# QZ1-boy/FCVSR

Hardware: AMD Instinct MI355X
Metric: SR frames/sec (7-frame window, 4x 180x320->720x1280) + PSNR vs ref (higher is better)
Workload: dtype bf16

## Files before the change

fcvsr_amd/csrc/iac.hip:

```cpp
#include "common.h"
#include "mfma_util.h"

namespace fcvsr {

typedef __attribute__((ext_vector_type(4))) float f32x4v_t;

constexpr int kIY = 4, kIX = 16, kIC = 32;
constexpr int kIHX = kIX + 2, kIHY = kIY + 2;

template <int KDT>
__device__ __forceinline__ void load_k12(const void* base, long long elem_off, float k[4][3]) {
  if (KDT == FCVSR_F32) {
    const float4* p = reinterpret_cast<const float4*>(reinterpret_cast<const float*>(base) + elem_off);
    const float4 a = p[0], b = p[1], c = p[2];
    k[0][0] = a.x; k[0][1] = a.y; k[0][2] = a.z; k[1][0] = a.w; k[1][1] = b.x; k[1][2] = b.y;
    k[2][0] = b.z; k[2][1] = b.w; k[2][2] = c.x; k[3][0] = c.y; k[3][1] = c.z; k[3][2] = c.w;
  } else {
    const uint2* p = reinterpret_cast<const uint2*>(reinterpret_cast<const uint16_t*>(base) + elem_off);
    const uint2 a = p[0], b = p[1], c = p[2];
    const unsigned w[6] = {a.x, a.y, b.x, b.y, c.x, c.y};
    float f[12];
#pragma unroll
    for (int i = 0; i < 6; ++i) {
      if (KDT == FCVSR_BF16) {
        f[2 * i] = __uint_as_float(w[i] << 16);
        f[2 * i + 1] = __uint_as_float(w[i] & 0xffff0000u);
      } else {
        typedef __attribute__((ext_vector_type(2))) _Float16 h2;
        const h2 hv = __builtin_bit_cast(h2, w[i]);
        f[2 * i] = (float)hv[0];
        f[2 * i + 1] = (float)hv[1];
      }
    }
#pragma unroll
    for (int c = 0; c < 4; ++c)
#pragma unroll
      for (int t = 0; t < 3; ++t) k[c][t] = f[c * 3 + t];
  }
}

template <int ADT>
__device__ __forceinline__ float4 ld_f4(const float* base, long long elem) {
  if (ADT == FCVSR_F32) return *reinterpret_cast<const float4*>(base + elem);
  const uint2 v = *reinterpret_cast<const uint2*>(reinterpret_cast<const uint16_t*>(base) + elem);
  if (ADT == FCVSR_BF16)
    return make_float4(__uint_as_float(v.x << 16), __uint_as_float(v.x & 0xffff0000u), __uint_as_float(v.y << 16),
                       __uint_as_float(v.y & 0xffff0000u));
  typedef __attribute__((ext_vector_type(2))) _Float16 h2;
  const h2 a = __builtin_bit_cast(h2, v.x), b = __builtin_bit_cast(h2, v.y);
  return make_float4((float)a[0], (float)a[1], (float)b[0], (float)b[1]);
}

template <int ADT>
__device__ __forceinline__ void st_f4(float* base, long long elem, float4 x) {
  if (ADT == FCVSR_F32) {
    *reinterpret_cast<float4*>(base + elem) = x;
  } else if (ADT == FCVSR_BF16) {
    typedef __attribute__((ext_vector_type(4))) __bf16 b4;
    const b4 c = {(__bf16)x.x, (__bf16)x.y, (__bf16)x.z, (__bf16)x.w};
    *reinterpret_cast<uint2*>(reinterpret_cast<uint16_t*>(base) + elem) = __builtin_bit_cast(uint2, c);
  } else {
    typedef __attribute__((ext_vector_type(4))) _Float16 h4;
    const h4 c = {(_Float16)x.x, (_Float16)x.y, (_Float16)x.z, (_Float16)x.w};
    *reinterpret_cast<uint2*>(reinterpret_cast<uint16_t*>(base) + elem) = __builtin_bit_cast(uint2, c);
  }
}

template <int KDT, int ADT>
__global__ __launch_bounds__(256) void iac_step_kernel(View prev, View off, View k1, View fin, float slope, int B, int H,
                                                       int W, View dst, int tiles_x, int tiles_y) {
  __shared__ __align__(16) float s_s[kIHY * kIHX * kIC];
  __shared__ __align__(16) float v_s[kIY * kIHX * kIC];
  const int tid = threadIdx.x;
  const int quad = tid & 7;
  const int c0 = blockIdx.y * kIC + quad * 4;
  const int t = blockIdx.x;
  const int b = t / (tiles_x * tiles_y);
  const int t2 = t - b * tiles_x * tiles_y;
  const int ty0 = (t2 / tiles_x) * kIY, tx0 = (t2 % tiles_x) * kIX;

  const long long pp = (long long)b * prev.sb + c0;
  for (int hp = tid >> 3; hp < kIHY * kIHX; hp += 32) {
    const int hy = hp / kIHX, hx = hp - hy * kIHX;
    int gy = ty0 + hy - 1, gx = tx0 + hx - 1;
    gy = gy < 0 ? 0 : (gy > H - 1 ? H - 1 : gy);
    gx = gx < 0 ? 0 : (gx > W - 1 ? W - 1 : gx);
    const float* op = off.p + (long long)b * off.sb + (long long)gy * off.sy + (long long)gx * off.sx;
    const float fx = (float)gx + op[0];
    const float fy = (float)gy + op[off.sc];
    const float x0f = floorf(fx), y0f = floorf(fy);
    const float wx1 = fx - x0f, wy1 = fy - y0f;
    const float wx0 = 1.f - wx1, wy0 = 1.f - wy1;
    const bool sane = (fx > -2.f) && (fx < (float)W + 1.f) && (fy > -2.f) && (fy < (float)H + 1.f);
    const int x0 = sane ? (int)x0f : -4, y0 = sane ? (int)y0f : -4;
    float4 acc = make_float4(0.f, 0.f, 0.f, 0.f);
#pragma unroll
    for (int dy = 0; dy < 2; ++dy) {
#pragma unroll
      for (int dx = 0; dx < 2; ++dx) {
        const int xi = x0 + dx, yi = y0 + dy;
        if (xi >= 0 && xi < W && yi >= 0 && yi < H) {
          const float w = (dy ? wy1 : wy0) * (dx ? wx1 : wx0);
          const float4 v = ld_f4<ADT>(prev.p, pp + (long long)yi * prev.sy + (long long)xi * prev.sx);
          acc.x = fmaf(v.x, w, acc.x); acc.y = fmaf(v.y, w, acc.y);
          acc.z = fmaf(v.z, w, acc.z); acc.w = fmaf(v.w, w, acc.w);
        }
      }
    }
    *reinterpret_cast<float4*>(s_s + hp * kIC + quad * 4) = acc;
  }
  __syncthreads();

  for (int vp = tid >> 3; vp < kIY * kIHX; vp += 32) {
    const int y = vp / kIHX, hx = vp - y * kIHX;
    int gy = ty0 + y, gx = tx0 + hx - 1;
    gy = gy > H - 1 ? H - 1 : gy;
    gx = gx < 0 ? 0 : (gx > W - 1 ? W - 1 : gx);
    float k[4][3];
    load_k12<KDT>(k1.p, (long long)b * k1.sb + (long long)gy * k1.sy + (long long)gx * k1.sx + c0 * 3, k);
    float4 acc = make_float4(0.f, 0.f, 0.f, 0.f);
#pragma unroll
    for (int tt = 0; tt < 3; ++tt) {
      const float4 v = *reinterpret_cast<const float4*>(s_s + ((y + tt) * kIHX + hx) * kIC + quad * 4);
      acc.x = fmaf(v.x, k[0][tt], acc.x); acc.y = fmaf(v.y, k[1][tt], acc.y);
      acc.z = fmaf(v.z, k[2][tt], acc.z); acc.w = fmaf(v.w, k[3][tt], acc.w);
    }
    *reinterpret_cast<float4*>(v_s + vp * kIC + quad * 4) = acc;
  }
  __syncthreads();

  for (int p = tid >> 3; p < kIY * kIX; p += 32) {
    const int y = p / kIX, x = p - y * kIX;
    const int gy = ty0 + y, gx = tx0 + x;
    if (gy < H && gx < W) {
      float k[4][3];
      load_k12<KDT>(k1.p, (long long)b * k1.sb + (long long)gy * k1.sy + (long long)gx * k1.sx + c0 * 3, k);
      float4 acc = make_float4(0.f, 0.f, 0.f, 0.f);
#pragma unroll
      for (int tt = 0; tt < 3; ++tt) {
        const float4 v = *reinterpret_cast<const float4*>(v_s + (y * kIHX + x + tt) * kIC + quad * 4);
        acc.x = fmaf(v.x, k[0][tt], acc.x); acc.y = fmaf(v.y, k[1][tt], acc.y);
        acc.z = fmaf(v.z, k[2][tt], acc.z); acc.w = fmaf(v.w, k[3][tt], acc.w);
      }
      const float4 f = ld_f4<ADT>(fin.p, (long long)b * fin.sb + (long long)gy * fin.sy + (long long)gx * fin.sx + c0);
      acc.x += f.x; acc.y += f.y; acc.z += f.z; acc.w += f.w;
      acc.x = acc.x >= 0.f ? acc.x : acc.x * slope; acc.y = acc.y >= 0.f ? acc.y : acc.y * slope;
      acc.z = acc.z >= 0.f ? acc.z : acc.z * slope; acc.w = acc.w >= 0.f ? acc.w : acc.w * slope;
      st_f4<ADT>(dst.p, (long long)b * dst.sb + (long long)gy * dst.sy + (long long)gx * dst.sx + c0, acc);
    }
  }
}

// ... 293 lines not shown
    for (int it = 0; it < NP; ++it) {
      const int src = dir * 32 + it * 8 + (lane >> 3);
#pragma unroll
      for (int q = 0; q < 4; ++q) {
        tap[dir][it][q] = ld_p8<ADT>(pb, __shfl(my_eo[q], src));
      }
    }
  };
  auto warp_store = [&](const int dir) {
#pragma unroll
    for (int it = 0; it < NP; ++it) {
      const int hp = it * 32 + ps;
      const int src = dir * 32 + it * 8 + (lane >> 3);
      float acc[8] = {0.f, 0.f, 0.f, 0.f, 0.f, 0.f, 0.f, 0.f};
      float tw[4];
#pragma unroll
      for (int q = 0; q < 4; ++q) tw[q] = __shfl(my_w[q], src);
#pragma unroll
      for (int q = 0; q < 4; ++q) {
        float v[8];
        unpack8<ADT>(tap[dir][it][q], v);
        const float w = tw[q];
#pragma unroll
        for (int c = 0; c < 8; ++c) acc[c] = fmaf(v[c], w, acc[c]);
      }
      if (hp < kIHY * kIHX) {
        *reinterpret_cast<float4*>(s_s + rec(hp, 0)) = make_float4(acc[0], acc[1], acc[2], acc[3]);
        *reinterpret_cast<float4*>(s_s + rec(hp, 1)) = make_float4(acc[4], acc[5], acc[6], acc[7]);
      }
    }
  };
  auto sac_phases = [&](const int dir) {
    const View dst = a.d[dir].dst;
#pragma unroll
    for (int j = 0; j < 3; ++j) {
      int y, hx;
      if (j < 2) { const int p = j * 32 + ps; y = p >> 4; hx = (p & 15) + 1; }
      else { y = ps >> 1; hx = (ps & 1) ? kIHX - 1 : 0; }
      if (j < 2 || ps < 8) {
        float k[24];
        unpack_k24<KDT>(j < 2 ? kin[j] : khal, k);
        float acc[8] = {0.f, 0.f, 0.f, 0.f, 0.f, 0.f, 0.f, 0.f};
#pragma unroll
        for (int tt = 0; tt < 3; ++tt) {
          const int sp = (y + tt) * kIHX + hx;
          const float4 va = *reinterpret_cast<const float4*>(s_s + rec(sp, 0)), vb = *reinterpret_cast<const float4*>(s_s + rec(sp, 1));
          const float v[8] = {va.x, va.y, va.z, va.w, vb.x, vb.y, vb.z, vb.w};
#pragma unroll
          for (int c = 0; c < 8; ++c) acc[c] = fmaf(v[c], k[c * 3 + tt], acc[c]);
        }
        const int vp = y * kIHX + hx;
        *reinterpret_cast<float4*>(v_s + rec(vp, 0)) = make_float4(acc[0], acc[1], acc[2], acc[3]);
        *reinterpret_cast<float4*>(v_s + rec(vp, 1)) = make_float4(acc[4], acc[5], acc[6], acc[7]);
      }
    }
    __syncthreads();
#pragma unroll
    for (int j = 0; j < 2; ++j) {
      const int p = j * 32 + ps;
      const int y = p >> 4, x = p & 15;
      const int gy = ty0 + y, gx = tx0 + x;
      if (gy < H && gx < W) {
        float k[24], f[8];
        unpack_k24<KDT>(kin[j], k);
        unpack8<ADT>(fpk[dir][j], f);
        float acc[8] = {0.f, 0.f, 0.f, 0.f, 0.f, 0.f, 0.f, 0.f};
#pragma unroll
        for (int tt = 0; tt < 3; ++tt) {
          const int vp = y * kIHX + x + tt;
          const float4 va = *reinterpret_cast<const float4*>(v_s + rec(vp, 0)), vb = *reinterpret_cast<const float4*>(v_s + rec(vp, 1));
          const float v[8] = {va.x, va.y, va.z, va.w, vb.x, vb.y, vb.z, vb.w};
#pragma unroll
          for (int c = 0; c < 8; ++c) acc[c] = fmaf(v[c], k[c * 3 + tt], acc[c]);
        }
#pragma unroll
        for (int c = 0; c < 8; ++c) {
          acc[c] += f[c];
          acc[c] = acc[c] >= 0.f ? acc[c] : acc[c] * slope;
        }
        st_p8<ADT>(dst.p, (long long)b * dst.sb + (long long)gy * dst.sy + (long long)gx * dst.sx + c0, acc);
      }
    }
  };

  issue_taps(0);
  if (FK) {
    predictor_gemm();
    __syncthreads();
#pragma unroll
    for (int j = 0; j < 2; ++j) {
      const int p = j * 32 + ps;
      const uint4* kq = reinterpret_cast<const uint4*>(kt_s + ((p >> 4) * kIHX + (p & 15) + 1) * kKtRow + oct * 24);
      kin[j].q[0] = kq[0]; kin[j].q[1] = kq[1]; kin[j].q[2] = kq[2];
    }
    if (ps < 8) {
      const uint4* kq = reinterpret_cast<const uint4*>(kt_s + ((ps >> 1) * kIHX + ((ps & 1) ? kIHX - 1 : 0)) * kKtRow + oct * 24);
      khal.q[0] = kq[0]; khal.q[1] = kq[1]; khal.q[2] = kq[2];
    }
    __syncthreads();
  }
  warp_store(0);
  if (ND > 1) { issue_taps(1); issue_fin(1); }
  if (t + 1 < t_end) off_next = load_off(t + 1, tid);
  __syncthreads();
  sac_phases(0);
  if (ND > 1) {
    warp_store(1);
    __syncthreads();
    sac_phases(1);
  }
  }
}


constexpr int kQX = 14, kQVX = 16, kQY = 4, kQSY = kQY + 2;
constexpr int kQNS = kQSY * kQVX, kQNV = kQY * kQVX;

template <bool BF16>
__device__ __forceinline__ f32x4v_t mfma16x(uint4 a, uint4 b, f32x4v_t c) {
  if (BF16)
    return __builtin_amdgcn_mfma_f32_16x16x32_bf16(__builtin_bit_cast(bf16x8_t, a), __builtin_bit_cast(bf16x8_t, b), c, 0, 0, 0);
  else
    return __builtin_amdgcn_mfma_f32_16x16x32_f16(__builtin_bit_cast(f16x8_t, a), __builtin_bit_cast(f16x8_t, b), c, 0, 0, 0);
}

struct Iac2Args {
  const uint16_t* prev[2];
  const float* off[2];
  const uint16_t* fin[2];
  uint16_t* dst[2];
  const uint16_t* k0;
  const uint16_t* wk;
  const float* kbias;
  long long prev_sb, off_sb, fin_sb, dst_sb, k0_sb;
  int prev_sy, prev_sx, off_sy, off_sx, off_sc, fin_sy, fin_sx, dst_sy, dst_sx, k0_sy, k0_sx;
  float slope;
  int H, W, tiles_x, tiles_y, ntiles;
};

#ifndef FCVSR_IAC2_WGS
#define FCVSR_IAC2_WGS 3
#endif
template <int KDT, int ADT>
__global__ __launch_bounds__(256, FCVSR_IAC2_WGS) void iac_fused2_kernel(Iac2Args a) {
  constexpr int NG = 1;
  static_assert(ADT != FCVSR_F32 && KDT != FCVSR_F32, "16-bit form");
  constexpr bool BF = KDT == FCVSR_BF16;
  constexpr int SPP = 32 * NG;
  constexpr int ND = 2, NP = (kQNS + SPP - 1) / SPP;
  constexpr int EARLY = 2;
  __shared__ __align__(16) float s_all[kQNS * kJC];
  __shared__ __align__(16) uint16_t w_s[3 * kJC * kJC];
  __shared__ __align__(16) float kb_s[3 * kJC];
  const float slope = a.slope;
  const int H = a.H, W = a.W, tiles_x = a.tiles_x, tiles_y = a.tiles_y;
  int t_begin, t_end;
  {
    const int g = blockIdx.x, nwg = gridDim.x, qq = nwg >> 3, rr = nwg & 7, xcd = g & 7, loc = g >> 3;
    const int ci = (xcd < rr ? xcd * (qq + 1) : rr * (qq + 1) + (xcd - rr) * qq) + loc;
    t_begin = (int)((long long)ci * a.ntiles / nwg);
    t_end = (int)((long long)(ci + 1) * a.ntiles / nwg);
  }
  {
    const int tid = threadIdx.x;
#pragma unroll
    for (int i = 0; i < 3 * kJC * kJC / 8 / (256 * NG); ++i) {
      const int idx = tid + 256 * NG * i, R = idx >> 3, seg = idx & 7;
      const int mt = R >> 4, r = R & 15, tp = mt >> 2, cb = mt & 3;
      const int orig = ((r >> 2) * 16 + cb * 4 + (r & 3)) * 3 + tp;
      *reinterpret_cast<uint4*>(w_s + R * kJC + ((seg ^ (R & 7)) << 3)) = *reinterpret_cast<const uint4*>(a.wk + orig * kJC + seg * 8);
    }
    if (tid < 3 * kJC) {
      const int mt = tid >> 4, r = tid & 15, tp = mt >> 2, cb = mt & 3;
      kb_s[tid] = a.kbias[((r >> 2) * 16 + cb * 4 + (r & 3)) * 3 + tp];
    }
    __syncthreads();
  }
  auto load_off = [&](const int tt, const int tidv) {
    const int lanev = tidv & 63, wavev = tidv >> 6;
    const int bb = tt / (tiles_x * tiles_y), tt2 = tt - bb * tiles_x * tiles_y;
    const int oy0 = (tt2 / tiles_x) * kQY, ox0 = (tt2 % tiles_x) * kQX;
    const int sdir = lanev >> 5, sit = (lanev >> 3) & 3, spl = lanev & 7;
    int hp = sit * SPP + wavev * 8 + spl;
    hp = hp < kQNS ? hp : kQNS - 1;
    const int hy = hp >> 4, hx = hp & 15;
    int gy = oy0 + hy - 1, gx = ox0 + hx - 1;
    gy = gy < 0 ? 0 : (gy > H - 1 ? H - 1 : gy);
    gx = gx < 0 ? 0 : (gx > W - 1 ? W - 1 : gx);
    const float* op = (sdir ? a.off[1] : a.off[0]) + (long long)bb * a.off_sb + (gy * a.off_sy + gx * a.off_sx);
    return make_float2(op[0], op[a.off_sc]);
  };
  const int wave_s = __builtin_amdgcn_readfirstlane((int)threadIdx.x >> 6);
  float* const s_s = s_all;
  float* const v_s = s_s;
  float2 off_next = make_float2(0.f, 0.f);
  if (t_begin < t_end) off_next = load_off(t_begin, (int)threadIdx.x);
  for (int t = t_begin; t < t_end; ++t) {
    int tid;
    asm volatile("v_mbcnt_lo_u32_b32 %0, -1, 0\n\tv_mbcnt_hi_u32_b32 %0, -1, %0\n\tv_lshl_add_u32 %0, %1, 6, %0" : "=&v"(tid) : "s"(wave_s));
    auto fresh = [&]() { int x = tid; asm volatile("" : "+v"(x)); return x; };
    const int wave = wave_s;
    const int b = t / (tiles_x * tiles_y);
    const int t2 = t - b * tiles_x * tiles_y;
    const int ty0 = (t2 / tiles_x) * kQY, tx0 = (t2 % tiles_x) * kQX;
    const int row = ty0 + wave;
    const int rowc = row > H - 1 ? H - 1 : row;
    auto col_of = [&](const int n_) { const int x = tx0 + n_ - 1; return x < 0 ? 0 : (x > W - 1 ? W - 1 : x); };
    auto ld16 = [](const void* base, const unsigned byte_off) {
      Pack8<ADT> r;
      r.a = *reinterpret_cast<const uint4*>(reinterpret_cast<const char*>(base) + byte_off);
      r.b = make_uint4(0, 0, 0, 0);
      return r;
    };
    uint4 kfr[2];
    {
      const int x = fresh(), n = x & 15, q = (x & 63) >> 4;
      const uint16_t* kb = a.k0 + (long long)b * a.k0_sb + (long long)rowc * a.k0_sy;
      const unsigned e = (unsigned)(col_of(n) * a.k0_sx + q * 8) * 2u;
      kfr[0] = ld16(kb, e).a;
      kfr[1] = ld16(kb, e + 64u).a;
    }
    int my_eo[4];
    float my_w[4];
    {
      const int x = fresh(), lane = x & 63;
      const int sit = (lane >> 3) & 3, spl = lane & 7;
      int hp = sit * SPP + wave * 8 + spl;
      hp = hp < kQNS ? hp : kQNS - 1;
      const int hy = hp >> 4, hx = hp & 15;
      int gy = ty0 + hy - 1, gx = tx0 + hx - 1;
      gy = gy < 0 ? 0 : (gy > H - 1 ? H - 1 : gy);
      gx = gx < 0 ? 0 : (gx > W - 1 ? W - 1 : gx);
      const int psy = a.prev_sy, psx = a.prev_sx;
      const float fx = (float)gx + off_next.x;
      const float fy = (float)gy + off_next.y;
      const float x0f = floorf(fx), y0f = floorf(fy);
      const float wx1 = fx - x0f, wy1 = fy - y0f;
      const float wx0 = 1.f - wx1, wy0 = 1.f - wy1;
      int wb, hb;
      asm volatile("v_mov_b32 %0, %2\n\tv_mov_b32 %1, %3" : "=&v"(wb), "=&v"(hb) : "s"(W + 1), "s"(H + 1));
      const bool sane = (fx > -2.f) && (fx < (float)wb) && (fy > -2.f) && (fy < (float)hb);
      const int x0 = sane ? (int)x0f : -4, y0 = sane ? (int)y0f : -4;
#pragma unroll
      for (int dy = 0; dy < 2; ++dy) {
#pragma unroll
        for (int dx = 0; dx < 2; ++dx) {
          const int xi = x0 + dx, yi = y0 + dy;
          const bool in = xi >= 0 && xi < W && yi >= 0 && yi < H;
          const int xc = xi < 0 ? 0 : (xi > W - 1 ? W - 1 : xi), yc = yi < 0 ? 0 : (yi > H - 1 ? H - 1 : yi);
          my_w[dy * 2 + dx] = in ? (dy ? wy1 : wy0) * (dx ? wx1 : wx0) : 0.f;
          my_eo[dy * 2 + dx] = yc * psy + xc * psx;
        }
      }
    }
    __builtin_amdgcn_sched_barrier(0);
    Pack8<ADT> fpk[2];
    auto issue_fin = [&](const int dir) {
      const int x = fresh(), n = x & 15, q = (x & 63) >> 4;
      const uint16_t* fb = a.fin[dir] + (long long)b * a.fin_sb + (long long)rowc * a.fin_sy;
      const unsigned e = (unsigned)(col_of(n) * a.fin_sx + q * 16) * 2u;
      fpk[0] = ld16(fb, e);
      fpk[1] = ld16(fb, e + 16u);
    };
    Pack8<ADT> tap[ND][NP][4];
    auto issue_taps = [&](const int dir, const int it0, const int it1) {
      const int x = fresh(), oct = x & 7, pull = ((x & 63) >> 3) << 2;
      const uint16_t* pb = a.prev[dir] + (long long)b * a.prev_sb;
#pragma unroll
      for (int it = it0; it < it1; ++it) {
        const int src = pull + dir * 128 + it * 32;
#pragma unroll
        for (int k = 0; k < 4; ++k)
          tap[dir][it][k] = ld16(pb, (unsigned)(__builtin_amdgcn_ds_bpermute(src, my_eo[k]) + oct * 8) * 2u);
      }
    };
    auto warp_store = [&](const int dir) {
      const int x = fresh(), oct = x & 7, ps = x >> 3, pull = ((x & 63) >> 3) << 2;
#pragma unroll
      for (int it = 0; it < NP; ++it) {
        const int hp = it * SPP + ps;
        const int src = pull + dir * 128 + it * 32;
        float acc[8] = {0.f, 0.f, 0.f, 0.f, 0.f, 0.f, 0.f, 0.f};
        float tw[4];
#pragma unroll
        for (int k = 0; k < 4; ++k) tw[k] = __int_as_float(__builtin_amdgcn_ds_bpermute(src, __float_as_int(my_w[k])));
#pragma unroll
        for (int k = 0; k < 4; ++k) {
          float v[8];
          unpack8<ADT>(tap[dir][it][k], v);
          const float w = tw[k];
#pragma unroll
          for (int c = 0; c < 8; ++c) acc[c] = fmaf(v[c], w, acc[c]);
        }
        float* rec = s_s + hp * kJC;
        if (kQNS % SPP == 0 || hp < kQNS) {
          *reinterpret_cast<float4*>(rec + (((2 * oct) ^ (hp & 15)) << 2)) = make_float4(acc[0], acc[1], acc[2], acc[3]);
          *reinterpret_cast<float4*>(rec + (((2 * oct + 1) ^ (hp & 15)) << 2)) = make_float4(acc[4], acc[5], acc[6], acc[7]);
        }
        __builtin_amdgcn_sched_barrier(0);
      }
    };
    issue_taps(0, 0, NP);
    __builtin_amdgcn_sched_barrier(0);
    constexpr bool KF = NG == 1 && BF;
    uint2 K1p[KF ? 1 : 12];
    float K1f[KF ? 12 : 1][4];
    {
      const int x = fresh(), n = x & 15, q = (x & 63) >> 4;
#pragma unroll
      for (int mt = 0; mt < 12; ++mt) {
        const int R = mt * 16 + n;
        const uint4 w0 = *reinterpret_cast<const uint4*>(w_s + R * kJC + ((q ^ (R & 7)) << 3));
        const uint4 w1 = *reinterpret_cast<const uint4*>(w_s + R * kJC + (((q + 4) ^ (R & 7)) << 3));
        f32x4v_t acc = {0.f, 0.f, 0.f, 0.f};
        acc = mfma16x<BF>(w0, kfr[0], acc);
        acc = mfma16x<BF>(w1, kfr[1], acc);
        const float4 b4 = *reinterpret_cast<const float4*>(kb_s + mt * 16 + q * 4);
        const uint2 pk = cvt4<BF>(make_float4(acc[0] + b4.x, acc[1] + b4.y, acc[2] + b4.z, acc[3] + b4.w));
        if (KF) cvt16x4_to_f32<BF>(pk, K1f[mt]);
        else K1p[mt] = pk;
        if (mt & 1) __builtin_amdgcn_sched_barrier(0);
      }
    }
    int ov[4], oh[3][4];
    {
      const int x = fresh(), n = x & 15, q = (x & 63) >> 4;
#pragma unroll
      for (int cb = 0; cb < 4; ++cb) {
        ov[cb] = n * kJC + (((q * 4 + cb) ^ n) << 2);
#pragma unroll
        for (int tt = 0; tt < 3; ++tt) {
          const int m = n + tt - 1;
          oh[tt][cb] = m * kJC + (((q * 4 + cb) ^ (m & 15)) << 2);
        }
      }
    }
    auto sac = [&](const int dir) {
      float4 vr[4];
      {
#pragma unroll
        for (int cb = 0; cb < 4; ++cb) {
          float acc[4] = {0.f, 0.f, 0.f, 0.f};
#pragma unroll
          for (int tt = 0; tt < 3; ++tt) {
            const float4 sv = *reinterpret_cast<const float4*>(s_s + (wave + tt) * (kQVX * kJC) + ov[cb]);
            float k[4];
            if (KF) { k[0] = K1f[tt * 4 + cb][0]; k[1] = K1f[tt * 4 + cb][1]; k[2] = K1f[tt * 4 + cb][2]; k[3] = K1f[tt * 4 + cb][3]; }
            else cvt16x4_to_f32<BF>(K1p[tt * 4 + cb], k);
            acc[0] = fmaf(sv.x, k[0], acc[0]); acc[1] = fmaf(sv.y, k[1], acc[1]);
            acc[2] = fmaf(sv.z, k[2], acc[2]); acc[3] = fmaf(sv.w, k[3], acc[3]);
          }
          vr[cb] = make_float4(acc[0], acc[1], acc[2], acc[3]);
          __builtin_amdgcn_sched_barrier(0);
        }
      }
      issue_fin(dir);
      __syncthreads();
#pragma unroll
      for (int cb = 0; cb < 4; ++cb) *reinterpret_cast<float4*>(v_s + wave * (kQVX * kJC) + ov[cb]) = vr[cb];
      __syncthreads();
      const int x = fresh(), n = x & 15, q = (x & 63) >> 4;
      const int gx = tx0 + n - 1;
      if (n >= 1 && n <= kQX && row < H && gx < W) {
        uint16_t* const db = a.dst[dir] + (long long)b * a.dst_sb + (long long)row * a.dst_sy;
        const int e = gx * a.dst_sx + q * 16;
#pragma unroll
        for (int hf = 0; hf < 2; ++hf) {
          float f[8], o[8];
          unpack8<ADT>(fpk[hf], f);
#pragma unroll
          for (int c2 = 0; c2 < 2; ++c2) {
            const int cb = hf * 2 + c2;
            float acc[4] = {0.f, 0.f, 0.f, 0.f};
#pragma unroll
            for (int tt = 0; tt < 3; ++tt) {
              const float4 vv = *reinterpret_cast<const float4*>(v_s + wave * (kQVX * kJC) + oh[tt][cb]);
              float k[4];
              if (KF) { k[0] = K1f[tt * 4 + cb][0]; k[1] = K1f[tt * 4 + cb][1]; k[2] = K1f[tt * 4 + cb][2]; k[3] = K1f[tt * 4 + cb][3]; }
              else cvt16x4_to_f32<BF>(K1p[tt * 4 + cb], k);
              acc[0] = fmaf(vv.x, k[0], acc[0]); acc[1] = fmaf(vv.y, k[1], acc[1]);
              acc[2] = fmaf(vv.z, k[2], acc[2]); acc[3] = fmaf(vv.w, k[3], acc[3]);
            }
#pragma unroll
            for (int i = 0; i < 4; ++i) {
              const float r = acc[i] + f[c2 * 4 + i];
              o[c2 * 4 + i] = fmaxf(r, r * slope);
            }
          }
          st_p8<ADT>(reinterpret_cast<float*>(db), e + hf * 8, o);
          __builtin_amdgcn_sched_barrier(0);
        }
      }
    };
    __builtin_amdgcn_sched_barrier(0);
    warp_store(0);
    __builtin_amdgcn_sched_barrier(0);
    issue_taps(1, 0, EARLY);
    __builtin_amdgcn_sched_barrier(0);
    __syncthreads();
    sac(0);
    issue_taps(1, EARLY, NP);
    if (t + 1 < t_end) off_next = load_off(t + 1, fresh());
    __builtin_amdgcn_sched_barrier(0);
    __syncthreads();
    warp_store(1);
    __syncthreads();
    sac(1);
    __syncthreads();
  }
}

}

using namespace fcvsr;

static bool quad_ok(const fcvsr_view* v, int dt) {
  if (!v || !v->ptr || v->dtype != dt || v->sc != 1 || v->c % 4) return false;
  const int g = dt == FCVSR_F32 ? 4 : 4;
  const int al = dt == FCVSR_F32 ? 16 : 8;
  return v->sx % g == 0 && v->sy % g == 0 && v->sb % g == 0 && ((uintptr_t)v->ptr % al) == 0;
}

static int iac_persistent_wgs() {
  static int n[64] = {0};
  int dev = 0;
  if (hipGetDevice(&dev) != hipSuccess || dev < 0 || dev >= 64) return 512;
  if (!n[dev]) {
    hipDeviceProp_t prop;
    n[dev] = hipGetDeviceProperties(&prop, dev) == hipSuccess && prop.multiProcessorCount > 0 ? 2 * prop.multiProcessorCount : 512;
  }
  return n[dev];
}

template <int KDT, int ND, bool FK = false>
static void launch_iac64(int adt, dim3 grid, hipStream_t st, IacArgs a) {
  a.ntiles = (int)grid.x;
  if (FK) {
    int nwg = iac_persistent_wgs() / (int)grid.y;
    nwg = nwg < 8 ? 8 : nwg / 8 * 8;
    if (nwg < (int)grid.x) grid.x = nwg;
  }
  if (adt == FCVSR_F32) hipLaunchKernelGGL((iac_step64_kernel<KDT, FCVSR_F32, ND, FK>), grid, dim3(256), 0, st, a);
  else if (adt == FCVSR_BF16) hipLaunchKernelGGL((iac_step64_kernel<KDT, FCVSR_BF16, ND, FK>), grid, dim3(256), 0, st, a);
  else hipLaunchKernelGGL((iac_step64_kernel<KDT, FCVSR_F16, ND, FK>), grid, dim3(256), 0, st, a);
}

template <int KDT>
static void launch_iac(int adt, bool wide, dim3 grid, hipStream_t st, View pv, View ov, View kv, View fv, float slope, int B, int H,
                       int W, View dv, int tx, int ty) {
  if (wide) {
    IacArgs a;
    a.d[0].prev = pv; a.d[0].off = ov; a.d[0].fin = fv; a.d[0].dst = dv;
    a.d[1] = a.d[0];
    a.k1 = kv; a.k0 = kv; a.wk = nullptr; a.kbias = nullptr; a.slope = slope; a.B = B; a.H = H; a.W = W; a.tiles_x = tx; a.tiles_y = ty;
    launch_iac64<KDT, 1>(adt, grid, st, a);
    return;
  }
  if (adt == FCVSR_F32)
    hipLaunchKernelGGL((iac_step_kernel<KDT, FCVSR_F32>), grid, dim3(256), 0, st, pv, ov, kv, fv, slope, B, H, W, dv, tx, ty);
  else if (adt == FCVSR_BF16)
    hipLaunchKernelGGL((iac_step_kernel<KDT, FCVSR_BF16>), grid, dim3(256), 0, st, pv, ov, kv, fv, slope, B, H, W, dv, tx, ty);
  else
    hipLaunchKernelGGL((iac_step_kernel<KDT, FCVSR_F16>), grid, dim3(256), 0, st, pv, ov, kv, fv, slope, B, H, W, dv, tx, ty);
}

extern "C" int fcvsr_iac_step(const fcvsr_view* prev, const fcvsr_view* off, const fcvsr_view* k1, const fcvsr_view* feat_in,
                              float slope, int B, int H, int W, const fcvsr_view* dst, void* stream) {
  FCVSR_CHECK_ARG(prev && prev->ptr, "null prev");
  const int adt = prev->dtype;
  FCVSR_CHECK_ARG(adt == FCVSR_F32 || adt == FCVSR_BF16 || adt == FCVSR_F16, "bad feature dtype");
  FCVSR_CHECK_ARG(quad_ok(prev, adt) && quad_ok(feat_in, adt) && quad_ok(dst, adt),
                  "prev/feat_in/dst: same dtype, channel-contiguous, aligned");
  FCVSR_CHECK_ARG(off && off->ptr && off->c >= 2 && off->dtype == FCVSR_F32, "off needs 2 f32 channels");
  FCVSR_CHECK_ARG(k1 && k1->ptr && k1->sc == 1 && k1->c == 3 * prev->c, "k1 must have 3*C contiguous channels");
  FCVSR_CHECK_ARG(prev->c % kIC == 0 && prev->c == dst->c && prev->c == feat_in->c, "C must be a multiple of 32");
  FCVSR_CHECK_ARG(B > 0 && H > 0 && W > 0, "bad sizes");
  const int g = k1->dtype == FCVSR_F32 ? 4 : 8;
  FCVSR_CHECK_ARG(((uintptr_t)k1->ptr % 16) == 0 && k1->sx % g == 0 && k1->sy % g == 0 && k1->sb % g == 0, "k1 alignment");
  const int tx = cdiv(W, kIX), ty = cdiv(H, kIY);
  const int fa = adt == FCVSR_F32 ? 4 : 8;
  auto wide_ok = [&](const fcvsr_view* v) { return ((uintptr_t)v->ptr % 16) == 0 && v->sx % fa == 0 && v->sy % fa == 0 && v->sb % fa == 0; };
  const bool wide = prev->c % kJC == 0 && wide_ok(prev) && wide_ok(feat_in) && wide_ok(dst) &&
                    (long long)H * prev->sy < (1ll << 31);
  dim3 grid(B * tx * ty, prev->c / (wide ? kJC : kIC));
  hipStream_t st = (hipStream_t)stream;
  const View pv = to_view(*prev), ov = to_view(*off), kv = to_view(*k1), fv = to_view(*feat_in), dv = to_view(*dst);
  if (k1->dtype == FCVSR_F32) launch_iac<FCVSR_F32>(adt, wide, grid, st, pv, ov, kv, fv, slope, B, H, W, dv, tx, ty);
  else if (k1->dtype == FCVSR_BF16) launch_iac<FCVSR_BF16>(adt, wide, grid, st, pv, ov, kv, fv, slope, B, H, W, dv, tx, ty);
  else launch_iac<FCVSR_F16>(adt, wide, grid, st, pv, ov, kv, fv, slope, B, H, W, dv, tx, ty);
  FCVSR_LAUNCH_CHECK();
  return 0;
}

extern "C" int fcvsr_iac_step2(const fcvsr_view* prev, const fcvsr_view* off, const fcvsr_view* k1, const fcvsr_view* feat_in,
                               float slope, int B, int H, int W, const fcvsr_view* dst, void* stream) {
  FCVSR_CHECK_ARG(prev && off && k1 && feat_in && dst && prev[0].ptr, "null argument");
  const int adt = prev[0].dtype;
  FCVSR_CHECK_ARG(adt == FCVSR_F32 || adt == FCVSR_BF16 || adt == FCVSR_F16, "bad feature dtype");
  const int fa = adt == FCVSR_F32 ? 4 : 8;
  for (int d = 0; d < 2; ++d) {
    FCVSR_CHECK_ARG(quad_ok(&prev[d], adt) && quad_ok(&feat_in[d], adt) && quad_ok(&dst[d], adt),
                    "prev/feat_in/dst: same dtype, channel-contiguous, aligned");
    FCVSR_CHECK_ARG(off[d].ptr && off[d].c >= 2 && off[d].dtype == FCVSR_F32, "off needs 2 f32 channels");
    FCVSR_CHECK_ARG(prev[d].c % kJC == 0 && prev[d].c == prev[0].c && prev[d].c == dst[d].c && prev[d].c == feat_in[d].c,
                    "C must be a multiple of 64 and alike for both directions");
    const fcvsr_view* vs[3] = {&prev[d], &feat_in[d], &dst[d]};
    for (const fcvsr_view* v : vs)
      FCVSR_CHECK_ARG(((uintptr_t)v->ptr % 16) == 0 && v->sx % fa == 0 && v->sy % fa == 0 && v->sb % fa == 0,
                      "16-byte aligned feature views");
  }
  FCVSR_CHECK_ARG(k1->ptr && k1->sc == 1 && k1->c == 3 * prev[0].c, "k1 must have 3*C contiguous channels");
  FCVSR_CHECK_ARG(B > 0 && H > 0 && W > 0, "bad sizes");
  const int g = k1->dtype == FCVSR_F32 ? 4 : 8;
  FCVSR_CHECK_ARG(((uintptr_t)k1->ptr % 16) == 0 && k1->sx % g == 0 && k1->sy % g == 0 && k1->sb % g == 0, "k1 alignment");
  const int tx = cdiv(W, kIX), ty = cdiv(H, kIY);
  dim3 grid(B * tx * ty, prev[0].c / kJC);
  IacArgs a;
  for (int d = 0; d < 2; ++d) {
    a.d[d].prev = to_view(prev[d]); a.d[d].off = to_view(off[d]); a.d[d].fin = to_view(feat_in[d]); a.d[d].dst = to_view(dst[d]);
  }
  a.k1 = to_view(*k1); a.k0 = a.k1; a.wk = nullptr; a.kbias = nullptr; a.slope = slope; a.B = B; a.H = H; a.W = W; a.tiles_x = tx; a.tiles_y = ty;
  hipStream_t st = (hipStream_t)stream;
  if (k1->dtype == FCVSR_F32) launch_iac64<FCVSR_F32, 2>(adt, grid, st, a);
  else if (k1->dtype == FCVSR_BF16) launch_iac64<FCVSR_BF16, 2>(adt, grid, st, a);
  else if (k1->dtype == FCVSR_F16) launch_iac64<FCVSR_F16, 2>(adt, grid, st, a);
  else FCVSR_CHECK_ARG(false, "bad k1 dtype");
  FCVSR_LAUNCH_CHECK();
  return 0;
}

extern "C" int fcvsr_iac_step2_fused(const fcvsr_view* prev, const fcvsr_view* off, const fcvsr_view* k0, const void* wk,
                                     const float* kbias, const fcvsr_view* feat_in, float slope, int B, int H, int W,
                                     const fcvsr_view* dst, void* stream) {
  FCVSR_CHECK_ARG(prev && off && k0 && wk && kbias && feat_in && dst && prev[0].ptr, "null argument");
  const int adt = prev[0].dtype;
  FCVSR_CHECK_ARG(adt == FCVSR_F32 || adt == FCVSR_BF16 || adt == FCVSR_F16, "bad feature dtype");
  const int fa = adt == FCVSR_F32 ? 4 : 8;
  for (int d = 0; d < 2; ++d) {
    FCVSR_CHECK_ARG(quad_ok(&prev[d], adt) && quad_ok(&feat_in[d], adt) && quad_ok(&dst[d], adt),
                    "prev/feat_in/dst: same dtype, channel-contiguous, aligned");
    FCVSR_CHECK_ARG(off[d].ptr && off[d].c >= 2 && off[d].dtype == FCVSR_F32, "off needs 2 f32 channels");
    FCVSR_CHECK_ARG(prev[d].c == kJC && dst[d].c == kJC && feat_in[d].c == kJC, "the fused predictor handles C == 64");
    const fcvsr_view* vs[3] = {&prev[d], &feat_in[d], &dst[d]};
    for (const fcvsr_view* v : vs)
      FCVSR_CHECK_ARG(((uintptr_t)v->ptr % 16) == 0 && v->sx % fa == 0 && v->sy % fa == 0 && v->sb % fa == 0,
                      "16-byte aligned feature views");
  }
  FCVSR_CHECK_ARG(k0->ptr && (k0->dtype == FCVSR_BF16 || k0->dtype == FCVSR_F16) && k0->sc == 1 && k0->c == kJC &&
                      ((uintptr_t)k0->ptr % 16) == 0 && k0->sx % 8 == 0 && k0->sy % 8 == 0 && k0->sb % 8 == 0,
                  "k0: 64 contiguous 16-bit channels, 16-byte aligned");
  FCVSR_CHECK_ARG(((uintptr_t)wk % 16) == 0 && ((uintptr_t)kbias % 16) == 0, "weights / bias must be 16-byte aligned");
  FCVSR_CHECK_ARG(B > 0 && H > 0 && W > 0, "bad sizes");
  FCVSR_CHECK_ARG((long long)H * prev[0].sy < (1ll << 31) && (long long)H * prev[1].sy < (1ll << 31), "image too large");
  const int tx = cdiv(W, kIX), ty = cdiv(H, kIY);
  dim3 grid(B * tx * ty, 1);
  IacArgs a;
  for (int d = 0; d < 2; ++d) {
    a.d[d].prev = to_view(prev[d]); a.d[d].off = to_view(off[d]); a.d[d].fin = to_view(feat_in[d]); a.d[d].dst = to_view(dst[d]);
  }
  a.k1 = to_view(*k0); a.k0 = to_view(*k0); a.wk = (const uint16_t*)wk; a.kbias = kbias;
  a.slope = slope; a.B = B; a.H = H; a.W = W; a.tiles_x = tx; a.tiles_y = ty;
// ... 33 lines not shown
```

fcvsr_amd/csrc/tail_fused.hip:

```cpp
#include "common.h"
#include "mfma_util.h"
#include "u8.h"

namespace fcvsr {

typedef __attribute__((ext_vector_type(4))) float f32x4_t;

constexpr int kTfTH = 8, kTfTW = 32;
constexpr int kTfHH = kTfTH + 2, kTfHW = kTfTW + 2;
constexpr int kTfNHP = kTfHH * kTfHW;
constexpr int kTfUH = kTfTH / 2 + 2, kTfUW = kTfTW / 2 + 2;
constexpr int kTfNU = kTfUH * kTfUW;
constexpr int kTfRow = 64 + 8;
constexpr int kTfPRow = 9;
constexpr int kTfNPT = (kTfNHP + 15) / 16;

struct TailArgs {
  View u1;
  const uint16_t* w2;
  const float* b2;
  const float* slope;
  const uint16_t* wl;
  const float* bl;
  View out;
  View out8;
  int B, H2, W2, tiles_x, tiles_y;
  int ntiles;
};

template <bool BF16>
__device__ __forceinline__ f32x4_t mfma16(uint4 a, uint4 b, f32x4_t c) {
  if (BF16)
    return __builtin_amdgcn_mfma_f32_16x16x32_bf16(__builtin_bit_cast(bf16x8_t, a), __builtin_bit_cast(bf16x8_t, b), c, 0, 0, 0);
  else
    return __builtin_amdgcn_mfma_f32_16x16x32_f16(__builtin_bit_cast(f16x8_t, a), __builtin_bit_cast(f16x8_t, b), c, 0, 0, 0);
}

template <bool BF16, int Q = 0>
__global__ __launch_bounds__(256, 3) void tail_fused_kernel(TailArgs a) {
  __shared__ __align__(16) uint16_t u2_s[kTfNHP * kTfRow];
  float* p_s = reinterpret_cast<float*>(u2_s);
  static_assert(kTfNPT * 16 * kTfPRow * 4 <= kTfNHP * kTfRow * 2, "tap table must fit into the u2 tile");
  __shared__ __align__(16) float b2_s[256];
  int t_begin, t_end;
  {
    const int g = blockIdx.x, nwg = gridDim.x, q = nwg >> 3, rr = nwg & 7, xcd = g & 7, loc = g >> 3;
    const int ci = (xcd < rr ? xcd * (q + 1) : rr * (q + 1) + (xcd - rr) * q) + loc;
    t_begin = (int)((long long)ci * a.ntiles / nwg);
    t_end = (int)((long long)(ci + 1) * a.ntiles / nwg);
  }
  uint4 wf[2][4], wl0, wl1;
  {
    const int tid0 = threadIdx.x, lane0 = tid0 & 63, wave0 = tid0 >> 6, r0 = lane0 & 31, h0 = lane0 >> 5;
#pragma unroll
    for (int q = 0; q < 2; ++q) {
      const uint16_t* wp = a.w2 + ((wave0 * 2 + q) * 32 + r0) * 64 + h0 * 8;
#pragma unroll
      for (int kk = 0; kk < 4; ++kk) wf[q][kk] = *reinterpret_cast<const uint4*>(wp + kk * 16);
    }
    wl0 = *reinterpret_cast<const uint4*>(a.wl + (lane0 & 15) * 64 + (lane0 >> 4) * 8);
    wl1 = *reinterpret_cast<const uint4*>(a.wl + (lane0 & 15) * 64 + (lane0 >> 4) * 8 + 32);
    b2_s[tid0] = a.b2 ? a.b2[tid0] : 0.f;
  }
  const float slope = a.slope[0];
  const float blast = a.bl ? a.bl[0] : 0.f;
  const int per_img = a.tiles_x * a.tiles_y;
  const int HH = 2 * a.H2, WW = 2 * a.W2;
  __syncthreads();
#pragma unroll 1
  for (int t = t_begin; t < t_end; ++t) {
  int tid = threadIdx.x;
  asm volatile("" : "+v"(tid));
  const int lane = tid & 63, wave = tid >> 6;
  const int b = t / per_img;
  const int t2 = t - b * per_img;
  const int Y0 = (t2 / a.tiles_x) * kTfTH, X0 = (t2 % a.tiles_x) * kTfTW;
  const int oy = Y0 + (tid >> 5), ox = X0 + (tid & 31);
  const bool olive = oy < HH && ox < WW;
  float* op = a.out.p + (long long)b * a.out.sb + (long long)(olive ? oy : 0) * a.out.sy + (long long)(olive ? ox : 0) * a.out.sx;
  const float base = *op;

  {
    const int r = lane & 31, h = lane >> 5;
    const uint16_t* ub = reinterpret_cast<const uint16_t*>(a.u1.p) + (long long)b * a.u1.sb + h * 8;
    uint4 kf[4][4];
#pragma unroll
    for (int nt = 0; nt < 4; ++nt) {
      int p = nt * 32 + r;
      p = p < kTfNU ? p : kTfNU - 1;
      const int uy = p / kTfUW, ux = p - uy * kTfUW;
      int gy = (Y0 >> 1) - 1 + uy, gx = (X0 >> 1) - 1 + ux;
      gy = gy < 0 ? 0 : (gy > a.H2 - 1 ? a.H2 - 1 : gy);
      gx = gx < 0 ? 0 : (gx > a.W2 - 1 ? a.W2 - 1 : gx);
      const uint16_t* up = ub + (long long)gy * a.u1.sy + (long long)gx * a.u1.sx;
#pragma unroll
      for (int kk = 0; kk < 4; ++kk) kf[nt][kk] = *reinterpret_cast<const uint4*>(up + kk * 16);
    }
    const int sy = wave >> 1, sx = wave & 1;
#pragma unroll
    for (int q = 0; q < 2; ++q) {
      float4 bq[4];
#pragma unroll
      for (int g = 0; g < 4; ++g)
        bq[g] = *reinterpret_cast<const float4*>(b2_s + wave * 64 + q * 32 + 8 * g + 4 * h);
#pragma unroll
      for (int nt = 0; nt < 4; ++nt) {
        f32x16_t acc;
#pragma unroll
        for (int i = 0; i < 16; ++i) acc[i] = 0.f;
#pragma unroll
        for (int kk = 0; kk < 4; ++kk) acc = mfma<BF16>(wf[q][kk], kf[nt][kk], acc);
        const int p = nt * 32 + r;
        const int uy = p / kTfUW, ux = p - uy * kTfUW;
        const int hr = 2 * uy + sy - 1, hc = 2 * ux + sx - 1;
        const int Y = Y0 - 1 + hr, X = X0 - 1 + hc;
        const bool keep = p < kTfNU && hr >= 0 && hr < kTfHH && hc >= 0 && hc < kTfHW;
        const bool inside = Y >= 0 && Y < HH && X >= 0 && X < WW;
#pragma unroll
        for (int g = 0; g < 4; ++g) {
          const int c = q * 32 + 8 * g + 4 * h;
          float4 v = make_float4(acc[4 * g] + bq[g].x, acc[4 * g + 1] + bq[g].y, acc[4 * g + 2] + bq[g].z, acc[4 * g + 3] + bq[g].w);
          v.x = fmaf(slope, fminf(v.x, 0.f), fmaxf(v.x, 0.f)); v.y = fmaf(slope, fminf(v.y, 0.f), fmaxf(v.y, 0.f));
          v.z = fmaf(slope, fminf(v.z, 0.f), fmaxf(v.z, 0.f)); v.w = fmaf(slope, fminf(v.w, 0.f), fmaxf(v.w, 0.f));
          uint2 pk = cvt4<BF16>(v);
          if (!inside) pk = make_uint2(0u, 0u);
          if (keep) *reinterpret_cast<uint2*>(u2_s + (hr * kTfHW + hc) * kTfRow + c) = pk;
        }
      }
    }
  }
  __syncthreads();

  {
    const int r16 = lane & 15, g4 = lane >> 4;
    f32x4_t pacc[(kTfNPT + 3) / 4];
#pragma unroll
    for (int j = 0; j < (kTfNPT + 3) / 4; ++j) {
      const int pt = wave + 4 * j;
      int px = pt * 16 + r16;
      px = px < kTfNHP ? px : kTfNHP - 1;
      const uint4 a0 = *reinterpret_cast<const uint4*>(u2_s + px * kTfRow + g4 * 8);
      const uint4 a1 = *reinterpret_cast<const uint4*>(u2_s + px * kTfRow + g4 * 8 + 32);
      f32x4_t acc = {0.f, 0.f, 0.f, 0.f};
      acc = mfma16<BF16>(a0, wl0, acc);
      pacc[j] = mfma16<BF16>(a1, wl1, acc);
    }
    __syncthreads();
#pragma unroll
    for (int j = 0; j < (kTfNPT + 3) / 4; ++j) {
      const int pt = wave + 4 * j;
      if (pt < kTfNPT && r16 < 9) {
#pragma unroll
        for (int i = 0; i < 4; ++i) p_s[(pt * 16 + 4 * g4 + i) * kTfPRow + r16] = pacc[j][i];
      }
    }
  }
  __syncthreads();

  {
    const int ty = tid >> 5, tx = tid & 31;
    if (olive) {
      float s = base + blast;
#pragma unroll
      for (int dy = 0; dy < 3; ++dy)
#pragma unroll
        for (int dx = 0; dx < 3; ++dx) s += p_s[((ty + dy) * kTfHW + tx + dx) * kTfPRow + dy * 3 + dx];
      if constexpr (Q == 0) {
        *op = s;
      } else {
        reinterpret_cast<uint8_t*>(a.out8.p)[(long long)b * a.out8.sb + (long long)oy * a.out8.sy + (long long)ox * a.out8.sx] =
            quantise_u8<Q>(s);
      }
    }
  }
  __syncthreads();
  }
}

}

using namespace fcvsr;

template <int Q>
static int tail_fused_launch(const fcvsr_view* u1, const void* w2, const float* b2, const float* slope, const void* wl, const float* bl,
                             int B, int H2, int W2, const fcvsr_view* out, const fcvsr_view* out8, void* stream) {
  FCVSR_CHECK_ARG(u1 && u1->ptr && w2 && slope && wl && out && out->ptr, "null argument");
  FCVSR_CHECK_ARG((u1->dtype == FCVSR_BF16 || u1->dtype == FCVSR_F16) && u1->c == 64 && u1->sc == 1 &&
                      ((uintptr_t)u1->ptr % 16) == 0 && u1->sx % 8 == 0 && u1->sy % 8 == 0 && u1->sb % 8 == 0,
                  "u1: 64 contiguous 16-bit channels, 16-byte aligned");
  FCVSR_CHECK_ARG(out->dtype == FCVSR_F32 && out->c == 1, "out: one f32 channel");
  FCVSR_CHECK_ARG(((uintptr_t)w2 % 16) == 0 && ((uintptr_t)wl % 16) == 0 && (b2 == nullptr || ((uintptr_t)b2 % 16) == 0),
                  "weights / bias must be 16-byte aligned");
  FCVSR_CHECK_ARG(B > 0 && H2 > 0 && W2 > 0, "bad sizes");
  TailArgs a;
  a.u1 = to_view(*u1); a.w2 = (const uint16_t*)w2; a.b2 = b2; a.slope = slope; a.wl = (const uint16_t*)wl; a.bl = bl;
  a.out = to_view(*out); a.B = B; a.H2 = H2; a.W2 = W2;
  a.out8 = out8 ? to_view(*out8) : a.out;
  a.tiles_x = cdiv(2 * W2, kTfTW);
  a.tiles_y = cdiv(2 * H2, kTfTH);
  a.ntiles = B * a.tiles_x * a.tiles_y;
  static int wgs[64] = {0};
  int dev = 0;
  if (hipGetDevice(&dev) != hipSuccess || dev < 0 || dev >= 64) dev = 0;
  if (!wgs[dev]) {
    hipDeviceProp_t prop;
    wgs[dev] = hipGetDeviceProperties(&prop, dev) == hipSuccess && prop.multiProcessorCount > 0 ? 3 * prop.multiProcessorCount : 768;
  }
  int nwg = wgs[dev];
  nwg = nwg < 8 ? 8 : nwg / 8 * 8;
  dim3 grid(nwg < a.ntiles ? nwg : a.ntiles);
  hipStream_t st = (hipStream_t)stream;
  if (u1->dtype == FCVSR_BF16) hipLaunchKernelGGL((tail_fused_kernel<true, Q>), grid, dim3(256), 0, st, a);
  else hipLaunchKernelGGL((tail_fused_kernel<false, Q>), grid, dim3(256), 0, st, a);
  FCVSR_LAUNCH_CHECK();
  return 0;
}

extern "C" int fcvsr_tail_fused(const fcvsr_view* u1, const void* w2, const float* b2, const float* slope, const void* wl,
                                const float* bl, int B, int H2, int W2, const fcvsr_view* out, void* stream) {
  return tail_fused_launch<0>(u1, w2, b2, slope, wl, bl, B, H2, W2, out, nullptr, stream);
}

extern "C" int fcvsr_tail_fused_u8(const fcvsr_view* u1, const void* w2, const float* b2, const float* slope, const void* wl,
                                   const float* bl, int B, int H2, int W2, const fcvsr_view* base, const fcvsr_view* out, int quantise,
                                   void* stream) {
  FCVSR_CHECK_ARG(out && out->ptr && out->dtype == FCVSR_U8 && out->c == 1, "out: one uint8 channel");
  FCVSR_CHECK_ARG(quantise == FCVSR_QUANT_TRUNCATE || quantise == FCVSR_QUANT_ROUND, "quantise: FCVSR_QUANT_TRUNCATE or _ROUND");
  if (quantise == FCVSR_QUANT_TRUNCATE)
    return tail_fused_launch<FCVSR_QUANT_TRUNCATE>(u1, w2, b2, slope, wl, bl, B, H2, W2, base, out, stream);
  return tail_fused_launch<FCVSR_QUANT_ROUND>(u1, w2, b2, slope, wl, bl, B, H2, W2, base, out, stream);
}
```

Measured before the change: 869.7.

## Walk tiles column-major and reuse overlapping halo rows between vertically adjacent tiles

Both the fused IAC kernel and the tail kernel now visit tiles in column-major order, so each workgroup processes vertically adjacent tiles one after another. When a tile continues from the previous one in the same column, the halo rows already computed are carried over instead of recomputed. In the IAC kernel they are held in registers (keep00..keep11) and written back into shared memory, and the first tap iteration is skipped. In the tail kernel the last two partial-product rows are copied to the top of p_s, and the first upsampling n-tile and the top pixel tiles are skipped. This removes redundant halo gathers and MFMA work, at the cost of more registers, extra branch variants, and a dependence on tile traversal order that could break correctness if the overlap assumptions are wrong.

```diff
diff --git a/fcvsr_amd/csrc/iac.hip b/fcvsr_amd/csrc/iac.hip
--- a/fcvsr_amd/csrc/iac.hip
+++ b/fcvsr_amd/csrc/iac.hip
@@ -1,3 +1,4 @@
+#include <type_traits>
 #include "common.h"
 #include "mfma_util.h"
 
@@ -597,6 +598,8 @@
   __shared__ __align__(16) float s_all[kQNS * kJC];
   __shared__ __align__(16) uint16_t w_s[3 * kJC * kJC];
   __shared__ __align__(16) float kb_s[3 * kJC];
+  float4 keep00, keep01, keep10, keep11;
+  keep00 = keep01 = keep10 = keep11 = make_float4(0.f, 0.f, 0.f, 0.f);
   const float slope = a.slope;
   const int H = a.H, W = a.W, tiles_x = a.tiles_x, tiles_y = a.tiles_y;
   int t_begin, t_end;
@@ -624,7 +627,8 @@
   auto load_off = [&](const int tt, const int tidv) {
     const int lanev = tidv & 63, wavev = tidv >> 6;
     const int bb = tt / (tiles_x * tiles_y), tt2 = tt - bb * tiles_x * tiles_y;
-    const int oy0 = (tt2 / tiles_x) * kQY, ox0 = (tt2 % tiles_x) * kQX;
+    const int txi = tt2 / tiles_y;
+    const int oy0 = (tt2 - txi * tiles_y) * kQY, ox0 = txi * kQX;
     const int sdir = lanev >> 5, sit = (lanev >> 3) & 3, spl = lanev & 7;
     int hp = sit * SPP + wavev * 8 + spl;
     hp = hp < kQNS ? hp : kQNS - 1;
@@ -640,14 +644,17 @@
   float* const v_s = s_s;
   float2 off_next = make_float2(0.f, 0.f);
   if (t_begin < t_end) off_next = load_off(t_begin, (int)threadIdx.x);
-  for (int t = t_begin; t < t_end; ++t) {
+  auto tile = [&](const int t, auto contc) __attribute__((always_inline)) {
+    constexpr bool CONT = decltype(contc)::value;
+    constexpr int P0 = CONT ? 1 : 0;
     int tid;
     asm volatile("v_mbcnt_lo_u32_b32 %0, -1, 0\n\tv_mbcnt_hi_u32_b32 %0, -1, %0\n\tv_lshl_add_u32 %0, %1, 6, %0" : "=&v"(tid) : "s"(wave_s));
     auto fresh = [&]() { int x = tid; asm volatile("" : "+v"(x)); return x; };
     const int wave = wave_s;
     const int b = t / (tiles_x * tiles_y);
     const int t2 = t - b * tiles_x * tiles_y;
-    const int ty0 = (t2 / tiles_x) * kQY, tx0 = (t2 % tiles_x) * kQX;
+    const int txi = t2 / tiles_y;
+    const int ty0 = (t2 - txi * tiles_y) * kQY, tx0 = txi * kQX;
     const int row = ty0 + wave;
     const int rowc = row > H - 1 ? H - 1 : row;
     auto col_of = [&](const int n_) { const int x = tx0 + n_ - 1; return x < 0 ? 0 : (x > W - 1 ? W - 1 : x); };
@@ -721,8 +728,14 @@
     };
     auto warp_store = [&](const int dir) {
       const int x = fresh(), oct = x & 7, ps = x >> 3, pull = ((x & 63) >> 3) << 2;
-#pragma unroll
-      for (int it = 0; it < NP; ++it) {
+      if (CONT) {
+        const int xi = fresh();
+        float4* s4 = reinterpret_cast<float4*>(s_s);
+        s4[xi] = dir ? keep10 : keep00;
+        s4[xi + 256] = dir ? keep11 : keep01;
+      }
+#pragma unroll
+      for (int it = P0; it < NP; ++it) {
         const int hp = it * SPP + ps;
         const int src = pull + dir * 128 + it * 32;
         float acc[8] = {0.f, 0.f, 0.f, 0.f, 0.f, 0.f, 0.f, 0.f};
@@ -745,7 +758,7 @@
         __builtin_amdgcn_sched_barrier(0);
       }
     };
-    issue_taps(0, 0, NP);
+    issue_taps(0, P0, NP);
     __builtin_amdgcn_sched_barrier(0);
     constexpr bool KF = NG == 1 && BF;
     uint2 K1p[KF ? 1 : 12];
@@ -799,6 +812,12 @@
           __builtin_amdgcn_sched_barrier(0);
         }
       }
+      {
+        const int xi = fresh();
+        const float4* s4 = reinterpret_cast<const float4*>(s_s + kQY * kQVX * kJC);
+        if (dir) { keep10 = s4[xi]; keep11 = s4[xi + 256]; }
+        else { keep00 = s4[xi]; keep01 = s4[xi + 256]; }
+      }
       issue_fin(dir);
       __syncthreads();
 #pragma unroll
@@ -840,11 +859,12 @@
     __builtin_amdgcn_sched_barrier(0);
     warp_store(0);
     __builtin_amdgcn_sched_barrier(0);
-    issue_taps(1, 0, EARLY);
+    constexpr int PE = P0 + EARLY < NP ? P0 + EARLY : NP;
+    issue_taps(1, P0, PE);
     __builtin_amdgcn_sched_barrier(0);
     __syncthreads();
     sac(0);
-    issue_taps(1, EARLY, NP);
+    issue_taps(1, PE, NP);
     if (t + 1 < t_end) off_next = load_off(t + 1, fresh());
     __builtin_amdgcn_sched_barrier(0);
     __syncthreads();
@@ -852,6 +872,11 @@
     __syncthreads();
     sac(1);
     __syncthreads();
+  };
+  for (int t = t_begin; t < t_end; ++t) {
+    const int t2 = t % (tiles_x * tiles_y);
+    if (t > t_begin && t2 % tiles_y != 0) tile(t, std::true_type{});
+    else tile(t, std::false_type{});
   }
 }
 
diff --git a/fcvsr_amd/csrc/tail_fused.hip b/fcvsr_amd/csrc/tail_fused.hip
--- a/fcvsr_amd/csrc/tail_fused.hip
+++ b/fcvsr_amd/csrc/tail_fused.hip
@@ -14,6 +14,7 @@
 constexpr int kTfRow = 64 + 8;
 constexpr int kTfPRow = 9;
 constexpr int kTfNPT = (kTfNHP + 15) / 16;
+constexpr int kTfNPTC = (kTfNHP - 2 * kTfHW + 15) / 16;
 
 struct TailArgs {
   View u1;
@@ -74,7 +75,9 @@
   const int lane = tid & 63, wave = tid >> 6;
   const int b = t / per_img;
   const int t2 = t - b * per_img;
-  const int Y0 = (t2 / a.tiles_x) * kTfTH, X0 = (t2 % a.tiles_x) * kTfTW;
+  const int txi = t2 / a.tiles_y, tyi = t2 - txi * a.tiles_y;
+  const int Y0 = tyi * kTfTH, X0 = txi * kTfTW;
+  const bool cont = t > t_begin && tyi != 0;
   const int oy = Y0 + (tid >> 5), ox = X0 + (tid & 31);
   const bool olive = oy < HH && ox < WW;
   float* op = a.out.p + (long long)b * a.out.sb + (long long)(olive ? oy : 0) * a.out.sy + (long long)(olive ? ox : 0) * a.out.sx;
@@ -83,10 +86,11 @@
   {
     const int r = lane & 31, h = lane >> 5;
     const uint16_t* ub = reinterpret_cast<const uint16_t*>(a.u1.p) + (long long)b * a.u1.sb + h * 8;
+    const int p0 = cont ? kTfUW : 0, hr0 = cont ? 2 : 0;
     uint4 kf[4][4];
 #pragma unroll
     for (int nt = 0; nt < 4; ++nt) {
-      int p = nt * 32 + r;
+      int p = p0 + nt * 32 + r;
       p = p < kTfNU ? p : kTfNU - 1;
       const int uy = p / kTfUW, ux = p - uy * kTfUW;
       int gy = (Y0 >> 1) - 1 + uy, gx = (X0 >> 1) - 1 + ux;
@@ -97,24 +101,17 @@
       for (int kk = 0; kk < 4; ++kk) kf[nt][kk] = *reinterpret_cast<const uint4*>(up + kk * 16);
     }
     const int sy = wave >> 1, sx = wave & 1;
-#pragma unroll
-    for (int q = 0; q < 2; ++q) {
-      float4 bq[4];
-#pragma unroll
-      for (int g = 0; g < 4; ++g)
-        bq[g] = *reinterpret_cast<const float4*>(b2_s + wave * 64 + q * 32 + 8 * g + 4 * h);
-#pragma unroll
-      for (int nt = 0; nt < 4; ++nt) {
+    auto ntile = [&](const int q, const int nt, const float4 (&bq)[4]) {
         f32x16_t acc;
 #pragma unroll
         for (int i = 0; i < 16; ++i) acc[i] = 0.f;
 #pragma unroll
         for (int kk = 0; kk < 4; ++kk) acc = mfma<BF16>(wf[q][kk], kf[nt][kk], acc);
-        const int p = nt * 32 + r;
+        const int p = p0 + nt * 32 + r;
         const int uy = p / kTfUW, ux = p - uy * kTfUW;
         const int hr = 2 * uy + sy - 1, hc = 2 * ux + sx - 1;
         const int Y = Y0 - 1 + hr, X = X0 - 1 + hc;
-        const bool keep = p < kTfNU && hr >= 0 && hr < kTfHH && hc >= 0 && hc < kTfHW;
+        const bool keep = p < kTfNU && hr >= hr0 && hr < kTfHH && hc >= 0 && hc < kTfHW;
         const bool inside = Y >= 0 && Y < HH && X >= 0 && X < WW;
 #pragma unroll
         for (int g = 0; g < 4; ++g) {
@@ -126,6 +123,24 @@
           if (!inside) pk = make_uint2(0u, 0u);
           if (keep) *reinterpret_cast<uint2*>(u2_s + (hr * kTfHW + hc) * kTfRow + c) = pk;
         }
+    };
+    auto bias_of = [&](const int q, float4 (&bq)[4]) {
+#pragma unroll
+      for (int g = 0; g < 4; ++g) bq[g] = *reinterpret_cast<const float4*>(b2_s + wave * 64 + q * 32 + 8 * g + 4 * h);
+    };
+#pragma unroll
+    for (int q = 0; q < 2; ++q) {
+      float4 bq[4];
+      bias_of(q, bq);
+#pragma unroll
+      for (int nt = 0; nt < 3; ++nt) ntile(q, nt, bq);
+    }
+    if (!cont) {
+#pragma unroll
+      for (int q = 0; q < 2; ++q) {
+        float4 bq[4];
+        bias_of(q, bq);
+        ntile(q, 3, bq);
       }
     }
   }
@@ -133,11 +148,14 @@
 
   {
     const int r16 = lane & 15, g4 = lane >> 4;
+    const int px0 = cont ? 2 * kTfHW : 0, npt = cont ? kTfNPTC : kTfNPT;
     f32x4_t pacc[(kTfNPT + 3) / 4];
 #pragma unroll
     for (int j = 0; j < (kTfNPT + 3) / 4; ++j) {
+      pacc[j] = f32x4_t{0.f, 0.f, 0.f, 0.f};
+      if (4 * j >= npt) break;
       const int pt = wave + 4 * j;
-      int px = pt * 16 + r16;
+      int px = px0 + pt * 16 + r16;
       px = px < kTfNHP ? px : kTfNHP - 1;
       const uint4 a0 = *reinterpret_cast<const uint4*>(u2_s + px * kTfRow + g4 * 8);
       const uint4 a1 = *reinterpret_cast<const uint4*>(u2_s + px * kTfRow + g4 * 8 + 32);
@@ -149,9 +167,9 @@
 #pragma unroll
     for (int j = 0; j < (kTfNPT + 3) / 4; ++j) {
       const int pt = wave + 4 * j;
-      if (pt < kTfNPT && r16 < 9) {
-#pragma unroll
-        for (int i = 0; i < 4; ++i) p_s[(pt * 16 + 4 * g4 + i) * kTfPRow + r16] = pacc[j][i];
+      if (pt < npt && r16 < 9) {
+#pragma unroll
+        for (int i = 0; i < 4; ++i) p_s[(px0 + pt * 16 + 4 * g4 + i) * kTfPRow + r16] = pacc[j][i];
       }
     }
   }
@@ -171,6 +189,16 @@
         reinterpret_cast<uint8_t*>(a.out8.p)[(long long)b * a.out8.sb + (long long)oy * a.out8.sy + (long long)ox * a.out8.sx] =
             quantise_u8<Q>(s);
       }
+    }
+    if (t + 1 < t_end && tyi + 1 < a.tiles_y && wave == 0) {
+      constexpr int kKeep4 = 2 * kTfHW * kTfPRow / 4;
+      static_assert(2 * kTfHW * kTfPRow % 4 == 0 && kTfTH * kTfHW * kTfPRow % 4 == 0, "kept rows are whole float4s");
+      static_assert(2 * kTfHW * kTfPRow * 4 <= kTfHW * kTfRow * 2, "kept rows must lie inside u2's halo row 0");
+      const float4* src = reinterpret_cast<const float4*>(p_s + kTfTH * kTfHW * kTfPRow);
+      float4* dst = reinterpret_cast<float4*>(p_s);
+#pragma unroll
+      for (int i = 0; i < (kKeep4 + 63) / 64; ++i)
+        if (lane + 64 * i < kKeep4) dst[lane + 64 * i] = src[lane + 64 * i];
     }
   }
   __syncthreads();
```

New measurement: 878.3 (median of 6 runs). Within noise of the previous version (+1.0%).
